# tigarcia/firedancer

Measured on AMD Instinct MI355X. Metric: ed25519 verifies/sec at 1/8 GPUs; % INT32 VALU roofline; p99 batch latency, higher is better.
Workload: dtype int32

## Files before the change

### firedancer_amd/csrc/fd_ed25519_kernels.hip

```cpp
#include <hip/hip_runtime.h>
#include "fd25519_dsm.h"
#include "fd25519_ge4.h"
#include "fd25519_sc.h"
#include "fd_sha512_dev.h"
#define FD_HALF_FN __device__ static inline
#define FD_HALF_RCP(y) __builtin_amdgcn_rcp(y)
#define FD_HALF_RCPF(y) __builtin_amdgcn_rcpf(y)
#include "fd25519_half.h"



#define FD_PF_FAIL  1u
#define FD_PF_SMALL 2u
#define FD_HF_DNEG  1u
#define FD_HF_FULL  2u


FD_DEV uint32_t nblk_bucket(uint32_t sz) {
  const uint32_t b = (sz + 208u) >> 7;
  return b < (FD_ED25519_SORT_BUCKETS - 1) ? b : (FD_ED25519_SORT_BUCKETS - 1);
}

#define FD_SORT_PER_THREAD 16
#define FD_SORT_PER_BLOCK (256 * FD_SORT_PER_THREAD)

FD_DEV uint32_t sort_wave_count(uint32_t* cnt, uint32_t b, bool valid) {
  const uint32_t lane = threadIdx.x & 63u;
  uint64_t active = __ballot(valid);
  uint32_t r = 0;
  while (active) {
    const int lead = __ffsll((unsigned long long)active) - 1;
    const uint32_t bl = (uint32_t)__shfl((int)b, lead);
    const uint64_t grp = __ballot(valid && b == bl) & active;
    uint32_t off = 0;
    if ((int)lane == lead) off = atomicAdd(&cnt[bl], (uint32_t)__popcll(grp));
    off = (uint32_t)__shfl((int)off, lead);
    if ((grp >> lane) & 1ull) r = off + (uint32_t)__popcll(grp & ((1ull << lane) - 1ull));
    active &= ~grp;
  }
  return r;
}

__global__ void __launch_bounds__(256) fd_ed25519_sort_hist_kernel(fd_ed25519_verify_params_t p) {
  __shared__ uint32_t h[FD_ED25519_SORT_BUCKETS];
  if (threadIdx.x < FD_ED25519_SORT_BUCKETS) h[threadIdx.x] = 0;
  __syncthreads();
  const uint64_t j0 = (uint64_t)blockIdx.x * FD_SORT_PER_BLOCK + threadIdx.x;
#pragma unroll
  for (int e = 0; e < FD_SORT_PER_THREAD; e++) {
    const uint64_t j = j0 + (uint64_t)e * 256u;
    const bool v = j < p.n;
    sort_wave_count(h, v ? nblk_bucket(p.msg_sz[p.base + j]) : 0u, v);
  }
  __syncthreads();
  if (threadIdx.x < FD_ED25519_SORT_BUCKETS && h[threadIdx.x]) atomicAdd(&p.hist[threadIdx.x], h[threadIdx.x]);
}

#ifndef FD_ED25519_SORT_DESC
#define FD_ED25519_SORT_DESC 1
#endif

__global__ void fd_ed25519_sort_scan_kernel(fd_ed25519_verify_params_t p) {
  if (threadIdx.x == 0) {
    uint32_t acc = 0;
    for (int i = 0; i < FD_ED25519_SORT_BUCKETS; i++) {
      const int b = FD_ED25519_SORT_DESC ? FD_ED25519_SORT_BUCKETS - 1 - i : i;
      p.hist[FD_ED25519_SORT_BUCKETS + b] = acc;
      acc += p.hist[b];
    }
  }
}

__global__ void __launch_bounds__(256) fd_ed25519_sort_scatter_kernel(fd_ed25519_verify_params_t p) {
  __shared__ uint32_t cnt[FD_ED25519_SORT_BUCKETS], base[FD_ED25519_SORT_BUCKETS];
  if (threadIdx.x < FD_ED25519_SORT_BUCKETS) cnt[threadIdx.x] = 0;
  __syncthreads();
  const uint64_t j0 = (uint64_t)blockIdx.x * FD_SORT_PER_BLOCK + threadIdx.x;
  uint32_t b[FD_SORT_PER_THREAD], r[FD_SORT_PER_THREAD];
#pragma unroll
  for (int e = 0; e < FD_SORT_PER_THREAD; e++) {
    const uint64_t j = j0 + (uint64_t)e * 256u;
    const bool v = j < p.n;
    b[e] = v ? nblk_bucket(p.msg_sz[p.base + j]) : 0u;
    r[e] = sort_wave_count(cnt, b[e], v);
  }
  __syncthreads();
  if (threadIdx.x < FD_ED25519_SORT_BUCKETS && cnt[threadIdx.x])
    base[threadIdx.x] = atomicAdd(&p.hist[FD_ED25519_SORT_BUCKETS + threadIdx.x], cnt[threadIdx.x]);
  __syncthreads();
#pragma unroll
  for (int e = 0; e < FD_SORT_PER_THREAD; e++) {
    const uint64_t j = j0 + (uint64_t)e * 256u;
    if (j < p.n) p.perm[base[b[e]] + r[e]] = (uint32_t)j;
  }
}

FD_DEV void hash_finish(const fd_ed25519_verify_params_t& p, uint64_t j, const uint32_t (&dig)[16],
                        const uint32_t (&S)[8]) {
  uint32_t k[8];
  sc_reduce512(k, dig);
#pragma unroll
  for (int w = 0; w < 8; w++) p.k[(uint64_t)w * p.cap + j] = k[w];
  p.sflag[j] = sc_is_canonical(S) ? 1 : 0;
}

FD_DEV void hash_one(const fd_ed25519_verify_params_t& p, uint64_t j) {
  const uint64_t i = p.base + j;
  uint32_t r[8], S[8], a[8];
  {
    const uint4* sg = reinterpret_cast<const uint4*>(p.sigs + 64 * i);
    const uint4* pk = reinterpret_cast<const uint4*>(p.pubs + 32 * i);
    const uint4 q0 = sg[0], q1 = sg[1], q2 = sg[2], q3 = sg[3], q4 = pk[0], q5 = pk[1];
    r[0] = q0.x; r[1] = q0.y; r[2] = q0.z; r[3] = q0.w; r[4] = q1.x; r[5] = q1.y; r[6] = q1.z; r[7] = q1.w;
    S[0] = q2.x; S[1] = q2.y; S[2] = q2.z; S[3] = q2.w; S[4] = q3.x; S[5] = q3.y; S[6] = q3.z; S[7] = q3.w;
    a[0] = q4.x; a[1] = q4.y; a[2] = q4.z; a[3] = q4.w; a[4] = q5.x; a[5] = q5.y; a[6] = q5.z; a[7] = q5.w;
  }
  uint32_t dig[16];
  if (p.digests) {
    const uint4* dg = reinterpret_cast<const uint4*>(p.digests + 64 * i);
#pragma unroll
    for (int q = 0; q < 4; q++) {
      const uint4 v = dg[q];
      dig[4 * q] = v.x; dig[4 * q + 1] = v.y; dig[4 * q + 2] = v.z; dig[4 * q + 3] = v.w;
    }
  } else {
    const uintptr_t mp = reinterpret_cast<uintptr_t>(p.msgs + p.msg_off[i]);
    sha_msg_src m;
    m.base = reinterpret_cast<const uint32_t*>(mp & ~(uintptr_t)3);
    m.shift = (uint32_t)(mp & 3);
    m.sz = p.msg_sz[i];
    sha512_ram(dig, r, a, m);
  }
  hash_finish(p, j, dig, S);
}

__global__ void __launch_bounds__(256, FD_ED25519_HASH_WAVES_PER_SIMD)
fd_ed25519_hash_kernel(fd_ed25519_verify_params_t p) {
  const uint64_t t = (uint64_t)blockIdx.x * blockDim.x + threadIdx.x;
  if (t >= p.n) return;
  hash_one(p, p.perm ? (uint64_t)p.perm[t] : t);
}

FD_DEV void decode_one(const fd_ed25519_verify_params_t& p, int which , uint64_t j) {
  const uint64_t i = p.base + j;
  uint32_t s[8];
  {
    const uint4* src = which ? reinterpret_cast<const uint4*>(p.sigs + 64 * i)
                             : reinterpret_cast<const uint4*>(p.pubs + 32 * i);
    const uint4 q0 = src[0], q1 = src[1];
    s[0] = q0.x; s[1] = q0.y; s[2] = q0.z; s[3] = q0.w; s[4] = q1.x; s[5] = q1.y; s[6] = q1.z; s[7] = q1.w;
  }
  decoded_pt d;
  ge_decode(d, s, !p.codes_portable);
  int32_t* dst = p.pts + (uint64_t)which * 20 * p.cap + j;
#pragma unroll
  for (int l = 0; l < 10; l++) {
    dst[(uint64_t)l * p.cap] = d.x.v[l];
    dst[(uint64_t)(10 + l) * p.cap] = d.y.v[l];
  }
  p.pflag[(uint64_t)which * p.cap + j] = (uint8_t)((d.fail ? FD_PF_FAIL : 0u) | (d.small ? FD_PF_SMALL : 0u));
}

__global__ void __launch_bounds__(256, FD_ED25519_DECODE_WAVES_PER_SIMD)
fd_ed25519_decode_kernel(fd_ed25519_verify_params_t p) {
  const uint64_t t = (uint64_t)blockIdx.x * blockDim.x + threadIdx.x;
  if (t >= 2 * p.n) return;
  const int which = t >= p.n;
  decode_one(p, which, which ? t - p.n : t);
}

FD_DEV void load_fe(fe& x, const int32_t* src, uint64_t cap) {
#pragma unroll
  for (int l = 0; l < 10; l++) x.v[l] = src[(uint64_t)l * cap];
}

FD_DEV void load_pt(fe& x, fe& y, const fd_ed25519_verify_params_t& p, int which, uint64_t j) {
  const int32_t* src = p.pts + (uint64_t)which * 20 * p.cap + j;
  load_fe(x, src, p.cap);
  load_fe(y, src + 10 * p.cap, p.cap);
}

#define FD_PENDING 1
FD_DEV int precheck(const fd_ed25519_verify_params_t& p, uint64_t j) {
  const uint32_t s_ok = p.sflag[j];
  const uint32_t af = p.pflag[j], rf = p.pflag[p.cap + j];
  if (!s_ok) return FD_ED25519_ERR_SIG;
  if (af & FD_PF_FAIL) return p.codes_portable ? FD_ED25519_ERR_PUBKEY : FD_ED25519_ERR_SIG;
  if (rf & FD_PF_FAIL) return FD_ED25519_ERR_SIG;
  if (af & FD_PF_SMALL) return FD_ED25519_ERR_PUBKEY;
  if (rf & FD_PF_SMALL) return FD_ED25519_ERR_SIG;
  return FD_PENDING;
}

template <bool NT>
FD_DEV void table_store(int4* tab, int e, ge_cached c) {
  if (NT) fe_neg(c.T2d, c.T2d);
  atab_store(tab, e, c);
}

__device__ const int4 fd_ident_cached[10] = {{1, 0, 0, 0}, {0, 0, 0, 0}, {0, 0, 1, 0}, {0, 0, 0, 0}, {0, 0, 0, 0},
                                             {2, 0, 0, 0}, {0, 0, 0, 0}, {0, 0, 0, 0}, {0, 0, 0, 0}, {0, 0, 0, 0}};

template <bool NT>
FD_DEV void table_build(int4* tab, const fe& x, const fe& y, bool negate) {
  ge_p3 P0;
  fe xn;
  fe_neg(xn, x);
  fe_select(P0.X, x, xn, negate);
  P0.Y = y;
  fe_1(P0.Z);
  fe_mul(P0.T, P0.X, y);
  ge_cached c1, c;
  c.YplusX = P0.Z; c.YminusX = P0.Z; fe_add(c.Z2, P0.Z, P0.Z); fe_0(c.T2d);
  atab_store(tab, 0, c);
  ge_p3_to_cached(c1, P0);
  table_store<NT>(tab, 1, c1);
  ge_precomp pre;
  pre.yplusx = c1.YplusX; pre.yminusx = c1.YminusX; pre.xy2d = c1.T2d;
  ge_p3 cur = P0;
  ge_p1p1 sum;
#pragma clang loop unroll(disable)
  for (int e = 2; e <= 8; e++) {
    ge_madd(sum, cur, pre);
    ge_p1p1_to_p3_uxyt(cur, sum);
    ge_p3_to_cached<true>(c, cur);
    table_store<NT>(tab, e, c);
  }
}

FD_DEV void table_add(ge_p1p1& Rt, const ge_p3& P, const int4* tab, int e) {
  ge_cached c;
  atab_load(c, tab, e < 0 ? -e : e);
  ge_cached_cneg(c, e < 0);
  ge_add(Rt, P, c);
}

FD_DEV void btab_add(ge_p1p1& Rt, const ge_p3& P, ge_precomp& b, int f) {
  ge_precomp_cneg(b, f < 0);
  ge_madd(Rt, P, b);
}


FD_DEV bool half_pair_ok(const uint32_t (&k)[8], const uint32_t (&c)[FD_HALF_TW], const uint32_t (&dm)[FD_HALF_TW],
                         int dneg, int dbits) {
  uint32_t x[16];
#pragma unroll
  for (int w = 0; w < 16; w++) x[w] = 0u;
#pragma unroll
  for (int a = 0; a < FD_HALF_TW; a++) {
    uint64_t carry = 0;
#pragma unroll
    for (int b = 0; b < 8; b++) {
      const uint64_t t = (uint64_t)dm[a] * k[b] + x[a + b] + carry;
      x[a + b] = (uint32_t)t;
      carry = t >> 32;
    }
    x[a + 8] = (uint32_t)carry;
  }
  const uint32_t n8l[8] = FD_HALF_N8L;
  uint32_t add[8];
  {
    uint64_t br = 0;
#pragma unroll
    for (int w = 0; w < 8; w++) {
      const uint32_t cv = w < FD_HALF_TW ? c[w] : 0u;
      const uint64_t t = (uint64_t)n8l[w] - cv - br;
      br = (t >> 63) & 1u;
      add[w] = dneg ? cv : (uint32_t)t;
    }
  }
  {
    uint64_t carry = 0;
#pragma unroll
    for (int w = 0; w < 15; w++) {
      const uint64_t t = (uint64_t)x[w] + (w < 8 ? add[w] : 0u) + carry;
      x[w] = (uint32_t)t;
      carry = t >> 32;
    }
  }
  const uint32_t low = x[0] & 7u;
#pragma unroll
  for (int w = 0; w < 15; w++) x[w] = __builtin_amdgcn_alignbit(x[w + 1], x[w], 3);
  x[15] >>= 3;
  uint32_t r[8];
  sc_reduce512(r, x);
  uint32_t nz = low;
#pragma unroll
  for (int w = 0; w < 8; w++) nz |= r[w];
  return nz == 0u && (dm[0] & 1u) && fd_half_bitlen<FD_HALF_TW>(c) <= FD_HALF_BITS &&
         fd_half_bitlen<FD_HALF_TW>(dm) <= dbits;
}

#ifndef FD_ED25519_HALF_FAULT
#define FD_ED25519_HALF_FAULT 0
#endif

FD_DEV int half_scalars_checked(const uint32_t (&k)[8], uint32_t (&c)[FD_HALF_TW], uint32_t (&dm)[FD_HALF_TW],
                                int* dneg, int dbits, uint64_t tag) {
  const int found = fd_half_scalars(k, c, dm, dneg, dbits);
#if FD_ED25519_HALF_FAULT
  {
    const uint32_t h = (uint32_t)(tag * 0x9E3779B97F4A7C15ull >> 32);
    const uint32_t sel = h >> 29, w = (h >> 8) & 3u, b = h & 31u;
#pragma unroll
    for (int i = 0; i < 4; i++) {
      if (sel == 1u && i == (int)w) c[i] ^= 1u << b;
      if (sel == 2u && i == (int)w) dm[i] ^= (i == 0 && b == 0) ? 2u : (1u << b);
    }
  }
#else
  (void)tag;
#endif
  return found && half_pair_ok(k, c, dm, *dneg, dbits);
}


FD_DEV void scalar_one(const fd_ed25519_verify_params_t& p, uint64_t j) {
  const uint64_t i = p.base + j;
  uint32_t k[8], S[8];
#pragma unroll
  for (int w = 0; w < 8; w++) k[w] = p.k[(uint64_t)w * p.cap + j];
  {
    const uint4* sg = reinterpret_cast<const uint4*>(p.sigs + 64 * i);
    const uint4 q2 = sg[2], q3 = sg[3];
    S[0] = q2.x; S[1] = q2.y; S[2] = q2.z; S[3] = q2.w; S[4] = q3.x; S[5] = q3.y; S[6] = q3.z; S[7] = q3.w;
  }
  uint32_t cw[FD_HALF_TW], dm[FD_HALF_TW];
  int dneg = 0;
  int ok = half_scalars_checked(k, cw, dm, &dneg, p.half_dbits, j);
#pragma unroll
  for (int w = 0; w < FD_HALF_TW; w++) {
    cw[w] = ok ? cw[w] : 0u;
    dm[w] = ok ? dm[w] : (w == 0 ? 1u : 0u);
  }
  dneg = ok ? dneg : 0;
  if (!p.sflag[j]) ok = 1;

  uint32_t sp[8];
  {
    uint32_t prod[16];
#pragma unroll
    for (int w = 0; w < 16; w++) prod[w] = 0u;
#pragma unroll
    for (int a = 0; a < FD_HALF_TW; a++) {
      uint64_t carry = 0;
#pragma unroll
      for (int b = 0; b < 8; b++) {
        const uint64_t t = (uint64_t)dm[a] * S[b] + prod[a + b] + carry;
        prod[a + b] = (uint32_t)t;
        carry = t >> 32;
      }
      prod[a + 8] = (uint32_t)carry;
    }
    sc_reduce512(sp, prod);
    if (dneg) {
      const uint32_t l[8] = {0x5cf5d3edu, 0x5812631au, 0xa2f79cd6u, 0x14def9deu, 0u, 0u, 0u, 0x10000000u};
      uint32_t nz = 0;
#pragma unroll
      for (int w = 0; w < 8; w++) nz |= sp[w];
      uint64_t br = 0;
#pragma unroll
      for (int w = 0; w < 8; w++) {
        const uint64_t t = (uint64_t)l[w] - sp[w] - br;
        br = (t >> 63) & 1u;
        sp[w] = nz ? (uint32_t)t : 0u;
      }
    }
  }
  uint32_t* hs = p.hs + j;
  const uint64_t c = p.cap;
  static_assert(FD_ED25519_BTABW_SHIFT == 144, "s_lo is words 0..3 and the low half of word 4");
#pragma unroll
  for (int w = 0; w < 5; w++) {
    hs[(uint64_t)w * c] = cw[w];
    hs[(uint64_t)(5 + w) * c] = dm[w];
    hs[(uint64_t)(10 + w) * c] = w < 4 ? sp[w] : (sp[4] & 0xffffu);
  }
#pragma unroll
  for (int w = 0; w < 4; w++)
    hs[(uint64_t)(15 + w) * c] = __builtin_amdgcn_alignbit(w + 5 < 8 ? sp[w + 5] : 0u, sp[w + 4], 16);
  p.hflag[j] = (uint8_t)((dneg ? FD_HF_DNEG : 0u) | (ok ? 0u : FD_HF_FULL));
  if (!ok && !p.small) {
    const uint32_t slot = atomicAdd(p.fix_cnt, 1u);
    p.fix_list[slot] = (uint32_t)j;
  }
}

__global__ void __launch_bounds__(256, FD_ED25519_SCALAR_WAVES_PER_SIMD)
fd_ed25519_scalar_kernel(fd_ed25519_verify_params_t p) {
  const uint64_t j = (uint64_t)blockIdx.x * blockDim.x + threadIdx.x;
  if (j >= p.n) return;
  scalar_one(p, j);
}

__global__ void __launch_bounds__(192) fd_ed25519_prep_kernel(fd_ed25519_verify_params_t p) {
  const uint32_t w = threadIdx.x >> 6;
  const uint64_t t = (uint64_t)blockIdx.x * 64u + (threadIdx.x & 63u);
  if (t >= p.n) return;
  if (w == 0) {
    const uint64_t j = p.perm ? (uint64_t)p.perm[t] : t;
    hash_one(p, j);
    scalar_one(p, j);
  } else {
    decode_one(p, (int)w - 1, t);
  }
}


FD_DEV void load_hs(uint32_t (&x)[5], const fd_ed25519_verify_params_t& p, int row, int words, uint64_t j) {
#pragma unroll
  for (int w = 0; w < 5; w++) x[w] = w < words ? p.hs[(uint64_t)(row + w) * p.cap + j] : 0u;
}

template <int BITS>
FD_DEV int wave_windows(const uint32_t (&d)[5]) {
  static_assert(BITS == 2 || BITS == 4, "2-bit or 4-bit windows");
  constexpr int W0 = 132 / BITS;
  int W = W0;
  const int wl = (fd_half_bitlen<5>(d) + BITS) >> (BITS / 2);
#pragma unroll
  for (int w = W0 + 1; w <= (FD_HALF_DBITS_MAX + BITS) / BITS; w++) W += __ballot(wl >= w) != 0ull;
  return W;
}

template <int BW>
struct fd_bw {
  static constexpr int STEP   = BW / 4;
  static constexpr int LO_N   = FD_ED25519_BTABW_SHIFT / BW;
  static constexpr int HI_N   = (253 - FD_ED25519_BTABW_SHIFT + BW - 1) / BW;
  static constexpr int LO_SHL = 160 - LO_N * BW;
  static constexpr int HI_SHL = 160 - HI_N * BW;
  static_assert(BW % 4 == 0, "base digits start at window boundaries");
  static_assert(LO_N * BW == FD_ED25519_BTABW_SHIFT, "s_lo digits cover bits 0..SHIFT-1");
  static_assert(HI_N * BW >= 253 - FD_ED25519_BTABW_SHIFT, "s_hi digits cover s' >> SHIFT");
  static_assert(STEP * (LO_N - 1) <= 32, "every base digit falls within the 33 windows");
  FD_DEV static bool lo_at(int it) { return it <= STEP * (LO_N - 1) && it % STEP == 0; }
  FD_DEV static bool hi_at(int it) { return it <= STEP * (HI_N - 1) && it % STEP == 0; }
};


FD_DEV void jtab_store(int4* tab, int slot, const ge_p3& P, bool neg) {
  ge_cached c;
  ge_p3_to_cached<true>(c, P);
  fe_neg(c.T2d, c.T2d);
  ge_cached_cneg(c, neg);
  atab_store(tab, slot, c);
}

FD_DEV void jtab_affine(ge_p3& P, const fd_ed25519_verify_params_t& p, int which, uint64_t j, bool negate) {
  fe x, xn;
  load_pt(x, P.Y, p, which, j);
  fe_neg(xn, x);
  fe_select(P.X, x, xn, negate);
  fe_1(P.Z);
  fe_mul(P.T, P.X, P.Y);
}

FD_DEV void jtab_step(int4* tab, int src, const ge_p3& q, int sp, int sm, bool mneg) {
  ge_cached e;
  atab_load(e, tab, src);
  fe qs, qd, m;
  fe_add(qs, q.Y, q.X);
  fe_sub(qd, q.Y, q.X);
  fe_mul(m, e.T2d, q.T);
#pragma clang loop unroll(disable)
  for (int h = sm < 0 ? 1 : 0; h < 2; h++) {
    const bool plus = h != 0;
    fe u, v, a, b, ms, mn;
    fe_select(u, qd, qs, plus);
    fe_select(v, qs, qd, plus);
    fe_mul_u(a, e.YplusX, u);
    fe_mul_u(b, e.YminusX, v);
    fe_neg(mn, m);
    fe_select(ms, mn, m, plus);
    ge_p1p1 sum;
    fe_sub(sum.X, a, b);
    fe_add(sum.Y, a, b);
    fe_sub(sum.Z, e.Z2, ms);
    fe_add(sum.T, e.Z2, ms);
    ge_p3 K;
    ge_p1p1_to_p3_uxyt(K, sum);
    jtab_store(tab, plus ? sp : sm, K, !plus && mneg);
  }
}

#define FD_JSLOT(a, r) (5 * (a) + (r) - 1)
FD_DEV void joint_table_build(int4* tab, const fd_ed25519_verify_params_t& p, uint64_t j, bool rneg) {
  ge_p3 P;
#pragma clang loop unroll(disable)
  for (int w = 0; w < 2; w++) {
    jtab_affine(P, p, w, j, w ? rneg : true);
    ge_cached c1;
    ge_p3_to_cached(c1, P);
    table_store<true>(tab, w ? FD_JSLOT(0, 1) : FD_JSLOT(1, 0), c1);
    ge_p1p1 sum;
    ge_p3_dbl(sum, P);
    ge_p3 D;
    ge_p1p1_to_p3_uxyt(D, sum);
    jtab_store(tab, w ? FD_JSLOT(0, 2) : FD_JSLOT(2, 0), D, false);
  }
#pragma clang loop unroll(disable)
  for (int st = 0; st < 4; st++) {
    const int src = st == 0 ? FD_JSLOT(0, 2) : st == 1 ? FD_JSLOT(1, 0) : st == 2 ? FD_JSLOT(2, 0) : FD_JSLOT(2, 1);
    const int sp = st == 0 ? FD_JSLOT(1, 2) : st == 1 ? FD_JSLOT(1, 1) : st == 2 ? FD_JSLOT(2, 1) : FD_JSLOT(2, 2);
    const int sm = st == 0 ? FD_JSLOT(1, -2) : st == 1 ? FD_JSLOT(1, -1) : st == 2 ? FD_JSLOT(2, -1) : -1;
    jtab_affine(P, p, st ? 1 : 0, j, st ? rneg : true);
    jtab_step(tab, src, P, sp, sm, st == 0);
  }
}

FD_DEV const int4* jtab_entry(const int4* tab, int a, int r) {
  const int slot = FD_JSLOT(a, r);
  return slot < 0 ? fd_ident_cached : tab + slot * 10;
}

template <int BW>
FD_DEV int dsm_half_one(const fd_ed25519_verify_params_t& p, uint64_t j, int4* tab) {
  int code = precheck(p, j);
  const uint32_t hf = p.hflag[j];
  joint_table_build(tab, p, j, !(hf & FD_HF_DNEG));
  uint32_t cd[5], dd[5], ld[5], hd[5];
  int W = 66;
  {
    uint32_t x[5], t[5];
    load_hs(x, p, 5, 5, j);
    const int wl = (fd_half_bitlen<5>(x) + 2) >> 1;
#pragma unroll
    for (int w = 67; w <= (FD_HALF_DBITS_MAX + 2) / 2; w++) W += __ballot(wl >= w) != 0ull;
    const int sh = 160 - 2 * W;
    shl160v(t, x, sh); recode160<2>(dd, t);
    load_hs(x, p, 0, 5, j);  shl160v(t, x, sh); recode160<2>(cd, t);
    load_hs(x, p, 10, 5, j); shl160<fd_bw<BW>::LO_SHL>(ld, x);
    load_hs(x, p, 15, 4, j); shl160<fd_bw<BW>::HI_SHL>(hd, x);
  }
  const int4* g_btab = reinterpret_cast<const int4*>(p.btab_lo);
  const int4* g_btab2 = reinterpret_cast<const int4*>(p.btab_hi);

  ge_p3 P;
  ge_p1p1 Rt;
  ge_p2 Q;
  {
    const int ea = pop160<2>(cd) & 3, er = pop160<2>(dd) & 3;
    ge_cached cj;
    atab_load(cj, jtab_entry(tab, ea, er), 0);
    fe t;
    fe_sub(t, cj.YplusX, cj.YminusX);
    fe_carry(Q.X, t);
    fe_add(t, cj.YplusX, cj.YminusX);
    fe_carry(Q.Y, t);
    Q.Z = cj.Z2;
  }
#pragma clang loop unroll(disable)
  for (int it = W - 2; it >= 0; it--) {
    const int ea = pop160<2>(cd), er = pop160<2>(dd);
    const bool sg = ea < 0 || (ea == 0 && er < 0);
    ge_cached cj;
    const bool blo = !(it & 1) && fd_bw<BW>::lo_at(it >> 1), bhi = !(it & 1) && fd_bw<BW>::hi_at(it >> 1);
    ge_precomp b1, b2;
    atab_load(cj, jtab_entry(tab, sg ? -ea : ea, sg ? -er : er), 0);
    if (blo) btab16_load(b1, g_btab, (int)pop160u<BW>(ld));
    if (bhi) btab16_load(b2, g_btab2, (int)pop160u<BW>(hd));
#pragma clang loop unroll(disable)
    for (int dbl = 0; dbl < 2; dbl++) {
      ge_p2_dbl(Rt, Q);
      if (dbl < 1) ge_p1p1_to_p2(Q, Rt);
    }
    ge_p1p1_to_p3_u(P, Rt);
    ge_cached_cneg(cj, sg);
    ge_add<true>(Rt, P, cj);
    if (blo) {
      ge_p1p1_to_p3_uxyt(P, Rt);
      ge_madd(Rt, P, b1);
    }
    if (bhi) {
      ge_p1p1_to_p3_uxyt(P, Rt);
      ge_madd(Rt, P, b2);
    }
    ge_p1p1_to_p2(Q, Rt);
  }
  fe t;
  fe_sub(t, Q.Y, Q.Z);
  const bool ident = fe_iszero(Q.X) && fe_iszero(t);
  if (code == FD_PENDING) code = ident ? FD_ED25519_SUCCESS : FD_ED25519_ERR_MSG;
  return code;
}

FD_DEV int dsm_full_core(const fd_ed25519_verify_params_t& p, uint64_t j, int4* tabA, int code, const fe& ax,
                         const fe& ay, const fe& rx, const fe& ry) {
  const uint64_t i = p.base + j;
  table_build<false>(tabA, ax, ay, true);
  uint32_t kd[8], sd[8];
  {
    uint32_t k[8], S[8];
#pragma unroll
    for (int w = 0; w < 8; w++) k[w] = p.k[(uint64_t)w * p.cap + j];
    const uint4* sg = reinterpret_cast<const uint4*>(p.sigs + 64 * i);
    const uint4 q2 = sg[2], q3 = sg[3];
    S[0] = q2.x; S[1] = q2.y; S[2] = q2.z; S[3] = q2.w; S[4] = q3.x; S[5] = q3.y; S[6] = q3.z; S[7] = q3.w;
    recode_radix16(kd, k);
    recode_radix65536(sd, S);
  }
  const int4* g_btab = reinterpret_cast<const int4*>(p.btab16);
  ge_p3 P;
  ge_p3_0(P);
  ge_p1p1 Rt;
  ge_p2 Q;
#pragma clang loop unroll(disable)
  for (int it = 63; it >= 0; it--) {
    const bool badd = (it & 3) == 0;
    int f = 0;
    ge_precomp b;
    if (badd) {
      f = pop_digit<16>(sd);
      btab16_load(b, g_btab, f < 0 ? -f : f);
    }
    if (it != 63) {
#pragma clang loop unroll(disable)
      for (int dbl = 0; dbl < 4; dbl++) {
        ge_p2_dbl(Rt, Q);
        if (dbl < 3) ge_p1p1_to_p2(Q, Rt);
      }
      ge_p1p1_to_p3_u(P, Rt);
    }
    table_add(Rt, P, tabA, pop_digit<4>(kd));
    if (badd) {
      ge_p1p1_to_p3_uxyt(P, Rt);
      btab_add(Rt, P, b, f);
    }
    ge_p1p1_to_p2(Q, Rt);
  }
  fe t1, t2;
  fe_mul(t1, rx, Q.Z);
  fe_sub(t1, t1, Q.X);
  fe_mul(t2, ry, Q.Z);
  fe_sub(t2, t2, Q.Y);
  const bool eq = fe_iszero(t1) && fe_iszero(t2);
  if (code != FD_PENDING) return code;
  return eq ? FD_ED25519_SUCCESS : FD_ED25519_ERR_MSG;
}

FD_DEV int dsm_full_one(const fd_ed25519_verify_params_t& p, uint64_t j, int4* tabA) {
  fe ax, ay, rx, ry;
  load_pt(ax, ay, p, 0, j);
  load_pt(rx, ry, p, 1, j);
  return dsm_full_core(p, j, tabA, precheck(p, j), ax, ay, rx, ry);
}

template <int BW>
__global__ void __launch_bounds__(FD_ED25519_VERIFY_BLOCK, FD_ED25519_DSM_WAVES_PER_SIMD)
fd_ed25519_dsm_kernel(fd_ed25519_verify_params_t p) {
  const uint32_t lane = threadIdx.x & 63u;
  const uint64_t wave = ((uint64_t)blockIdx.x * blockDim.x + threadIdx.x) >> 6;
  int4* tabA = reinterpret_cast<int4*>(static_cast<char*>(p.atab) + wave * FD_ED25519_ATAB_BYTES_PER_WAVE) +
               lane * (2 * FD_ED25519_ATAB_STRIDE * 10);
  if (p.small) {
    const uint64_t stride = (uint64_t)gridDim.x * blockDim.x;
    for (uint64_t t = (uint64_t)blockIdx.x * blockDim.x + threadIdx.x; t < p.n; t += stride)
      if (p.hflag[t] & FD_HF_FULL) p.out[p.base + t] = (int8_t)dsm_full_one(p, t, tabA);
    return;
  }
  const uint64_t nfix = *p.fix_cnt;
  const uint64_t head = (nfix + 63u) & ~(uint64_t)63u;
  const uint64_t total = head + p.n;
  for (;;) {
    uint32_t b = 0u;
    if (lane == 0u) b = atomicAdd(p.work_ctr, 64u);
    b = (uint32_t)__builtin_amdgcn_readfirstlane((int)__shfl((int)b, 0));
    if ((uint64_t)b >= total) break;
    const uint64_t t = (uint64_t)b + lane;
    if (t < nfix) {
      const uint64_t j = p.fix_list[t];
      p.out[p.base + j] = (int8_t)dsm_full_one(p, j, tabA);
    } else if (t >= head && t < total) {
      const uint64_t j = t - head;
      if (!(p.hflag[j] & FD_HF_FULL)) p.out[p.base + j] = (int8_t)dsm_half_one<BW>(p, j, tabA);
    }
  }
}


FD_DEV void tab4_store(int4* tab, int e, const fe& c) {
  int4* d = tab + 3 * e;
  d[0] = make_int4(c.v[0], c.v[1], c.v[2], c.v[3]);
  d[1] = make_int4(c.v[4], c.v[5], c.v[6], c.v[7]);
  d[2] = make_int4(c.v[8], c.v[9], 0, 0);
}

FD_DEV void tab4_load(fe& c, const int4* tab, int e) {
  const int4* s = tab + 3 * e;
  const int4 a = s[0], b = s[1], d = s[2];
  c.v[0] = a.x; c.v[1] = a.y; c.v[2] = a.z; c.v[3] = a.w;
  c.v[4] = b.x; c.v[5] = b.y; c.v[6] = b.z; c.v[7] = b.w;
  c.v[8] = d.x; c.v[9] = d.y;
}

FD_DEV void btab4_load(fe& c, const int32_t* g_btab, int e, const qmask_t& m) {
  const int off = m.l0 ? 10 : (m.l1 ? 0 : 20);
  const int2* s = reinterpret_cast<const int2*>(g_btab + (size_t)e * FD_ED25519_BTAB16_STRIDE + off);
#pragma unroll
  for (int q = 0; q < 5; q++) {
    const int2 x = s[q];
    c.v[2 * q] = x.x;
    c.v[2 * q + 1] = x.y;
  }
#pragma unroll
  for (int i = 0; i < 10; i++) c.v[i] = m.l3 ? (i == 0 ? 2 : 0) : c.v[i];
}

FD_DEV void table4_build(int4* tab, const fe& x, const fe& y, bool negate, const qmask_t& m) {
  fe xs, xy, p0, c1, c, r, cur;
#pragma unroll
  for (int i = 0; i < 10; i++) xs.v[i] = negate ? -x.v[i] : x.v[i];
  fe_mul(xy, xs, y);
#pragma unroll
  for (int i = 0; i < 10; i++) {
    p0.v[i] = m.l0 ? xs.v[i] : (m.l1 ? y.v[i] : (m.l2 ? (i == 0 ? 1 : 0) : xy.v[i]));
    c.v[i] = i == 0 ? (m.l2 ? 0 : (m.l3 ? 2 : 1)) : 0;
  }
  tab4_store(tab, 0, c);
  ge4_to_qc(c1, p0, m);
  tab4_store(tab, 1, c1);
  cur = p0;
#pragma clang loop unroll(disable)
  for (int e = 2; e <= 8; e++) {
    ge4_add(r, cur, c1, m);
    ge4_to_p3(cur, r);
    ge4_to_qc(c, cur, m);
    tab4_store(tab, e, c);
  }
}

FD_DEV void ge4_dbl4(fe& P, const qmask_t& m) {
  fe Rt;
#pragma clang loop unroll(disable)
  for (int dbl = 0; dbl < 4; dbl++) {
    ge4_dbl(Rt, P, m);
    ge4_to_p3(P, Rt);
  }
}

FD_DEV void ge4_add_signed(fe& P, const fe& c, bool neg, const qmask_t& m) {
  fe Rt;
  ge4_cneg(P, m.l03, neg);
  ge4_add(Rt, P, c, m);
  ge4_cneg(Rt, m.l0, neg);
  ge4_to_p3(P, Rt);
}

FD_DEV void quad_finish(const fd_ed25519_verify_params_t& p, uint64_t j, const fe& P, int code, bool store) {
  fe y1, z1, t;
  fe_qp<FD_QP(1, 1, 1, 1)>(y1, P);
  fe_qp<FD_QP(2, 2, 2, 2)>(z1, P);
  fe_sub(t, y1, z1);
  const bool ident = fe_iszero(P) && fe_iszero(t);
  if (code == FD_PENDING) code = ident ? FD_ED25519_SUCCESS : FD_ED25519_ERR_MSG;
  if (store) p.out[p.base + j] = (int8_t)code;
}

template <int BW>
__global__ void __launch_bounds__(256) fd_ed25519_dsm4_kernel(fd_ed25519_verify_params_t p) {
  const uint64_t gid = (uint64_t)blockIdx.x * blockDim.x + threadIdx.x;
  const uint64_t j = gid >> 2;
  if (j >= p.n) return;
  const uint32_t hf = p.hflag[j];
  if (hf & FD_HF_FULL) return;
  const qmask_t m = quad_masks();
  int4* tabA = reinterpret_cast<int4*>(static_cast<char*>(p.atab) + gid * FD_ED25519_QUAD_LANE_BYTES);
  int4* tabR = tabA + 27;
  int code = precheck(p, j);
  {
    fe x, y;
    load_pt(x, y, p, 0, j);
    table4_build(tabA, x, y, true, m);
    load_pt(x, y, p, 1, j);
    table4_build(tabR, x, y, !(hf & FD_HF_DNEG), m);
  }
  uint32_t cd[5], dd[5], ld[5], hd[5];
  int W;
  {
    uint32_t x[5], t[5];
    load_hs(x, p, 5, 5, j);
    W = wave_windows<4>(x);
    const int sh = 160 - 4 * W;
    shl160v(t, x, sh); recode160<4>(dd, t);
    load_hs(x, p, 0, 5, j);  shl160v(t, x, sh); recode160<4>(cd, t);
    load_hs(x, p, 10, 5, j); shl160<fd_bw<BW>::LO_SHL>(ld, x);
    load_hs(x, p, 15, 4, j); shl160<fd_bw<BW>::HI_SHL>(hd, x);
  }
  fe P, Rt;
#pragma unroll
  for (int i = 0; i < 10; i++) P.v[i] = (i == 0 && (m.l1 | m.l2)) ? 1 : 0;
#pragma clang loop unroll(disable)
  for (int it = W - 1; it >= 0; it--) {
    int ea = pop160<4>(cd), er = pop160<4>(dd);
    if (it == W - 1) { ea &= 15; er &= 15; }
    const bool blo = fd_bw<BW>::lo_at(it), bhi = fd_bw<BW>::hi_at(it);
    fe ca, cr, b1, b2;
    tab4_load(ca, tabA, ea < 0 ? -ea : ea);
    if (it != W - 1) ge4_dbl4(P, m);
    tab4_load(cr, tabR, er < 0 ? -er : er);
    ge4_add_signed(P, ca, ea < 0, m);
    if (blo) btab4_load(b1, p.btab_lo, (int)pop160u<BW>(ld), m);
    if (bhi) btab4_load(b2, p.btab_hi, (int)pop160u<BW>(hd), m);
    ge4_add_signed(P, cr, er < 0, m);
    if (blo) {
      ge4_add(Rt, P, b1, m);
      ge4_to_p3(P, Rt);
    }
    if (bhi) {
      ge4_add(Rt, P, b2, m);
      ge4_to_p3(P, Rt);
    }
  }
  quad_finish(p, j, P, code, m.l0);
}

template <int BW>
__global__ void __launch_bounds__(256) fd_ed25519_dsm8_kernel(fd_ed25519_verify_params_t p) {
  const uint64_t gid = (uint64_t)blockIdx.x * blockDim.x + threadIdx.x;
  const uint64_t j = gid >> 3;
  if (j >= p.n) return;
  const uint32_t hf = p.hflag[j];
  if (hf & FD_HF_FULL) return;
  const int half = (int)((threadIdx.x >> 2) & 1u);
  const qmask_t m = quad_masks();
  int4* tab = reinterpret_cast<int4*>(static_cast<char*>(p.atab) + gid * (FD_ED25519_QUAD_LANE_BYTES / 2));
  int code = precheck(p, j);
  {
    fe x, y;
    load_pt(x, y, p, half, j);
    table4_build(tab, x, y, half ? !(hf & FD_HF_DNEG) : true, m);
  }
  uint32_t sd[5], bd[5];
  int W;
  {
    uint32_t x[5], t[5];
    load_hs(x, p, 5, 5, j);
    W = wave_windows<4>(x);
    if (!half) load_hs(x, p, 0, 5, j);
    shl160v(t, x, 160 - 4 * W); recode160<4>(sd, t);
    if (half) {
      load_hs(x, p, 15, 4, j);
      shl160<fd_bw<BW>::HI_SHL>(bd, x);
    } else {
      load_hs(x, p, 10, 5, j);
      shl160<fd_bw<BW>::LO_SHL>(bd, x);
    }
  }
  const int32_t* btab = half ? p.btab_hi : p.btab_lo;
  fe P, Rt;
#pragma unroll
  for (int i = 0; i < 10; i++) P.v[i] = (i == 0 && (m.l1 | m.l2)) ? 1 : 0;
#pragma clang loop unroll(disable)
  for (int it = W - 1; it >= 0; it--) {
    int e = pop160<4>(sd);
    if (it == W - 1) e &= 15;
    const bool badd = half ? fd_bw<BW>::hi_at(it) : fd_bw<BW>::lo_at(it);
    fe ce, b;
    tab4_load(ce, tab, e < 0 ? -e : e);
    if (it != W - 1) ge4_dbl4(P, m);
    if (badd) btab4_load(b, btab, (int)pop160u<BW>(bd), m);
    ge4_add_signed(P, ce, e < 0, m);
// ... 684 lines not shown
```

Before: 107.9 million.

## Share Z coordinates across joint table entries and reuse affine point data

Restructures the joint A/R precompute table so entries that share a Z coordinate (affine points, and the minus-variants of each step) store only their first 30 ints, while a Z-map bitfield redirects Z loads to a shared slot. This skips the final Z multiplication for minus-variants. The two affine points are loaded and converted once and then reused, instead of being reloaded for every step. The identity entry is laid out to match the split layout. The intent is to cut field multiplies and global loads during table build. The cost is extra indirection and split loads in the hot main loop.

After: 108.7 million (median of 6 runs). About the same (+0.8%).

```diff
diff --git a/firedancer_amd/csrc/fd_ed25519_kernels.hip b/firedancer_amd/csrc/fd_ed25519_kernels.hip
--- a/firedancer_amd/csrc/fd_ed25519_kernels.hip
+++ b/firedancer_amd/csrc/fd_ed25519_kernels.hip
@@ -199,7 +199,7 @@
 }
 
 __device__ const int4 fd_ident_cached[10] = {{1, 0, 0, 0}, {0, 0, 0, 0}, {0, 0, 1, 0}, {0, 0, 0, 0}, {0, 0, 0, 0},
-                                             {2, 0, 0, 0}, {0, 0, 0, 0}, {0, 0, 0, 0}, {0, 0, 0, 0}, {0, 0, 0, 0}};
+                                             {0, 0, 0, 0}, {0, 0, 0, 0}, {0, 0, 2, 0}, {0, 0, 0, 0}, {0, 0, 0, 0}};
 
 template <bool NT>
 FD_DEV void table_build(int4* tab, const fe& x, const fe& y, bool negate) {
@@ -439,36 +439,104 @@
 };
 
 
-FD_DEV void jtab_store(int4* tab, int slot, const ge_p3& P, bool neg) {
+#define FD_JTAB_ZMAP 0xCBAB876067200ull
+#define FD_JTAB_Z_INT 30
+
+FD_DEV const int4* jtab_rows(const int4* tab, int slot) {
+  return slot < 0 ? fd_ident_cached : tab + slot * 10;
+}
+
+FD_DEV const int4* jtab_zrows(const int4* tab, int slot) {
+  return jtab_rows(tab, (int)((uint32_t)(FD_JTAB_ZMAP >> (4 * (slot + 1))) & 15u) - 1);
+}
+
+FD_DEV void jtab_store_head(int4* tab, int slot, const ge_cached& c) {
+  int v[30];
+#pragma unroll
+  for (int i = 0; i < 10; i++) {
+    v[i] = c.YplusX.v[i];
+    v[10 + i] = c.YminusX.v[i];
+    v[20 + i] = c.T2d.v[i];
+  }
+  int4* d = tab + slot * 10;
+#pragma unroll
+  for (int q = 0; q < 7; q++) d[q] = make_int4(v[4 * q], v[4 * q + 1], v[4 * q + 2], v[4 * q + 3]);
+  reinterpret_cast<int2*>(d)[FD_JTAB_Z_INT / 2 - 1] = make_int2(v[28], v[29]);
+}
+
+FD_DEV void jtab_store_z(int4* tab, int slot, const fe& z2) {
+  int4* d = tab + slot * 10;
+  reinterpret_cast<int2*>(d)[FD_JTAB_Z_INT / 2] = make_int2(z2.v[0], z2.v[1]);
+  d[8] = make_int4(z2.v[2], z2.v[3], z2.v[4], z2.v[5]);
+  d[9] = make_int4(z2.v[6], z2.v[7], z2.v[8], z2.v[9]);
+}
+
+FD_DEV void jtab_load(ge_cached& c, const int4* e, const int4* z) {
+  int v[40];
+#pragma unroll
+  for (int q = 0; q < 7; q++) {
+    const int4 x = e[q];
+    v[4 * q] = x.x; v[4 * q + 1] = x.y; v[4 * q + 2] = x.z; v[4 * q + 3] = x.w;
+  }
+  const int2 h = reinterpret_cast<const int2*>(e)[FD_JTAB_Z_INT / 2 - 1];
+  const int2 z0 = reinterpret_cast<const int2*>(z)[FD_JTAB_Z_INT / 2];
+  const int4 z1 = z[8], z2 = z[9];
+  v[28] = h.x; v[29] = h.y;
+  v[30] = z0.x; v[31] = z0.y;
+  v[32] = z1.x; v[33] = z1.y; v[34] = z1.z; v[35] = z1.w;
+  v[36] = z2.x; v[37] = z2.y; v[38] = z2.z; v[39] = z2.w;
+#pragma unroll
+  for (int i = 0; i < 10; i++) {
+    c.YplusX.v[i] = v[i];
+    c.YminusX.v[i] = v[10 + i];
+    c.T2d.v[i] = v[20 + i];
+    c.Z2.v[i] = v[30 + i];
+  }
+}
+
+FD_DEV void jtab_store(int4* tab, int slot, const ge_p3& P, bool neg, bool withz) {
   ge_cached c;
   ge_p3_to_cached<true>(c, P);
   fe_neg(c.T2d, c.T2d);
   ge_cached_cneg(c, neg);
-  atab_store(tab, slot, c);
-}
-
-FD_DEV void jtab_affine(ge_p3& P, const fd_ed25519_verify_params_t& p, int which, uint64_t j, bool negate) {
+  jtab_store_head(tab, slot, c);
+  if (withz) jtab_store_z(tab, slot, c.Z2);
+}
+
+struct jtab_q { fe ypx, ymx, T; };
+
+FD_DEV void jtab_affine(jtab_q& q, int4* tab, const fd_ed25519_verify_params_t& p, int which, uint64_t j, bool negate,
+                        int s1, int s2) {
+  ge_p3 P;
   fe x, xn;
   load_pt(x, P.Y, p, which, j);
   fe_neg(xn, x);
   fe_select(P.X, x, xn, negate);
   fe_1(P.Z);
   fe_mul(P.T, P.X, P.Y);
-}
-
-FD_DEV void jtab_step(int4* tab, int src, const ge_p3& q, int sp, int sm, bool mneg) {
+  ge_cached c1;
+  ge_p3_to_cached(c1, P);
+  q.ypx = c1.YplusX; q.ymx = c1.YminusX; q.T = P.T;
+  fe_neg(c1.T2d, c1.T2d);
+  jtab_store_head(tab, s1, c1);
+  ge_p1p1 sum;
+  ge_p3_dbl(sum, P);
+  ge_p3 D;
+  ge_p1p1_to_p3_uxyt(D, sum);
+  jtab_store(tab, s2, D, false, true);
+}
+
+FD_DEV void jtab_step(int4* tab, int src, const jtab_q& q, int sp, int sm, bool mneg) {
   ge_cached e;
-  atab_load(e, tab, src);
-  fe qs, qd, m;
-  fe_add(qs, q.Y, q.X);
-  fe_sub(qd, q.Y, q.X);
+  jtab_load(e, jtab_rows(tab, src), jtab_zrows(tab, src));
+  fe m;
   fe_mul(m, e.T2d, q.T);
 #pragma clang loop unroll(disable)
   for (int h = sm < 0 ? 1 : 0; h < 2; h++) {
     const bool plus = h != 0;
     fe u, v, a, b, ms, mn;
-    fe_select(u, qd, qs, plus);
-    fe_select(v, qs, qd, plus);
+    fe_select(u, q.ymx, q.ypx, plus);
+    fe_select(v, q.ypx, q.ymx, plus);
     fe_mul_u(a, e.YplusX, u);
     fe_mul_u(b, e.YminusX, v);
     fe_neg(mn, m);
@@ -479,39 +547,42 @@
     fe_sub(sum.Z, e.Z2, ms);
     fe_add(sum.T, e.Z2, ms);
     ge_p3 K;
-    ge_p1p1_to_p3_uxyt(K, sum);
-    jtab_store(tab, plus ? sp : sm, K, !plus && mneg);
+    fe x19, z19;
+    fe_19(x19, sum.X);
+    fe_19(z19, sum.Z);
+    fe_mul19_u(K.X, sum.T, sum.X, x19);
+    fe_mul19_u(K.T, sum.Y, sum.X, x19);
+    fe_mul19_u(K.Y, sum.Y, sum.Z, z19);
+    if (plus) fe_mul19(K.Z, sum.T, sum.Z, z19);
+    else K.Z = sum.Z;
+    jtab_store(tab, plus ? sp : sm, K, !plus && mneg, plus);
   }
 }
 
 #define FD_JSLOT(a, r) (5 * (a) + (r) - 1)
 FD_DEV void joint_table_build(int4* tab, const fd_ed25519_verify_params_t& p, uint64_t j, bool rneg) {
-  ge_p3 P;
+  jtab_q q, R1;
 #pragma clang loop unroll(disable)
-  for (int w = 0; w < 2; w++) {
-    jtab_affine(P, p, w, j, w ? rneg : true);
-    ge_cached c1;
-    ge_p3_to_cached(c1, P);
-    table_store<true>(tab, w ? FD_JSLOT(0, 1) : FD_JSLOT(1, 0), c1);
-    ge_p1p1 sum;
-    ge_p3_dbl(sum, P);
-    ge_p3 D;
-    ge_p1p1_to_p3_uxyt(D, sum);
-    jtab_store(tab, w ? FD_JSLOT(0, 2) : FD_JSLOT(2, 0), D, false);
+  for (int w = 1; w >= 0; w--) {
+    jtab_affine(q, tab, p, w, j, w ? rneg : true, w ? FD_JSLOT(0, 1) : FD_JSLOT(1, 0), w ? FD_JSLOT(0, 2) : FD_JSLOT(2, 0));
+    if (w) R1 = q;
   }
 #pragma clang loop unroll(disable)
   for (int st = 0; st < 4; st++) {
     const int src = st == 0 ? FD_JSLOT(0, 2) : st == 1 ? FD_JSLOT(1, 0) : st == 2 ? FD_JSLOT(2, 0) : FD_JSLOT(2, 1);
     const int sp = st == 0 ? FD_JSLOT(1, 2) : st == 1 ? FD_JSLOT(1, 1) : st == 2 ? FD_JSLOT(2, 1) : FD_JSLOT(2, 2);
     const int sm = st == 0 ? FD_JSLOT(1, -2) : st == 1 ? FD_JSLOT(1, -1) : st == 2 ? FD_JSLOT(2, -1) : -1;
-    jtab_affine(P, p, st ? 1 : 0, j, st ? rneg : true);
-    jtab_step(tab, src, P, sp, sm, st == 0);
+    if (st == 1) q = R1;
+    jtab_step(tab, src, q, sp, sm, st == 0);
   }
 }
 
 FD_DEV const int4* jtab_entry(const int4* tab, int a, int r) {
-  const int slot = FD_JSLOT(a, r);
-  return slot < 0 ? fd_ident_cached : tab + slot * 10;
+  return jtab_rows(tab, FD_JSLOT(a, r));
+}
+
+FD_DEV const int4* jtab_entry_z(const int4* tab, int a, int r) {
+  return jtab_zrows(tab, FD_JSLOT(a, r));
 }
 
 template <int BW>
@@ -542,7 +613,7 @@
   {
     const int ea = pop160<2>(cd) & 3, er = pop160<2>(dd) & 3;
     ge_cached cj;
-    atab_load(cj, jtab_entry(tab, ea, er), 0);
+    jtab_load(cj, jtab_entry(tab, ea, er), jtab_entry_z(tab, ea, er));
     fe t;
     fe_sub(t, cj.YplusX, cj.YminusX);
     fe_carry(Q.X, t);
@@ -557,7 +628,7 @@
     ge_cached cj;
     const bool blo = !(it & 1) && fd_bw<BW>::lo_at(it >> 1), bhi = !(it & 1) && fd_bw<BW>::hi_at(it >> 1);
     ge_precomp b1, b2;
-    atab_load(cj, jtab_entry(tab, sg ? -ea : ea, sg ? -er : er), 0);
+    jtab_load(cj, jtab_entry(tab, sg ? -ea : ea, sg ? -er : er), jtab_entry_z(tab, sg ? -ea : ea, sg ? -er : er));
     if (blo) btab16_load(b1, g_btab, (int)pop160u<BW>(ld));
     if (bhi) btab16_load(b2, g_btab2, (int)pop160u<BW>(hd));
 #pragma clang loop unroll(disable)
```
